# cv-core/MIT-Driverless-CV-TrainingInfra

Hardware: AMD Instinct MI355X
Metric: images/sec training (YOLOv3 416^2 + RektNet 80^2) (higher is better)
Workload: dtype bf16; 1 GPU; CVC-YOLOv3 yolo_baseline 416x416 classes=80, train step (fwd+bwd+Adam), 32 img/GPU; global_batch=32, parallelism=dp1, hipgraph=False, optimizer=FusedAdam

## Files before the change

mit-driverless-cv-traininginfra_amd/csrc/conv_igemm.hip:

```cpp
#include "conv_gemm.h"
#include "conv_shift.h"
#include "wgrad_gemm.h"
#include "wgrad_shift.h"
#include "wgrad_stream.h"

extern "C" {

static int conv2d_impl(int dtype, int mode, const void* in, int in_ldc, const void* w_packed, void* out, int out_ldc,
                       const float* bias, const void* addsrc, int add_ldc, float* stats_partial,
                       int B, int Hin, int Win, int Cin, int Hout, int Wout, int Nout,
                       int KH, int KW, int stride, int pad, int dil, const BnFuseArgs* fuse, void* stream, const EpiArgs* epi = nullptr,
                       const XAccArgs* xacc = nullptr) {
  if (!in || !w_packed || !out) return MDCV_EARG;
  if (xacc && (mode != 0 || stats_partial || fuse || epi || !xacc->acc || xacc->reps < 1 || (xacc->reps & (xacc->reps - 1)))) return MDCV_EARG;
  if (epi && (mode != 0 || stats_partial || fuse)) return MDCV_EARG;
  if ((Cin & 7) || (Nout & 7) || (in_ldc & 7) || (out_ldc & 7) || (addsrc && (add_ldc & 7))) return MDCV_EARG;
  if (stride != 1 && stride != 2) return MDCV_EARG;
  if (mode != 0 && mode != 1) return MDCV_EARG;
  ConvArgs a;
  a.in = in; a.w = w_packed; a.out = out; a.bias = bias; a.addsrc = addsrc; a.stats = stats_partial;
  a.in_ldc = in_ldc; a.out_ldc = out_ldc; a.add_ldc = add_ldc;
  a.Hin = Hin; a.Win = Win; a.Cin = Cin; a.Hout = Hout; a.Wout = Wout; a.Nout = Nout;
  a.KH = KH; a.KW = KW; a.stride = stride; a.pad = pad; a.dil = dil;
  a.M = B * Hout * Wout; a.Ktot = KH * KW * Cin; a.tiles_n = 0; a.sshift = stride == 2 ? 1 : 0; a.tiles_total = 0; a.xcd_chunk = 0;
// ... 50 lines not shown
    return dtype == MDCV_BF16 ? mdcv_cd_bf16_dgrad(a, st, B) : (dtype == MDCV_F32 ? mdcv_cd_f32_dgrad(a, st, B) : MDCV_EARG);
  }
  if (shift_ok && stats_partial) {
    const int r0 = cdiv(a.M, 128), r1 = mdcv_shift_fwd_stats_rows(B, Hout, Wout, Nout, dil);
    if (r1 > r0) {
      hipError_t e = hipMemsetAsync(stats_partial + (size_t)r0 * 2 * Nout, 0, (size_t)(r1 - r0) * 2 * Nout * sizeof(float), st);
      if (e != hipSuccess) return (int)e;
    }
  }
  if (dtype == MDCV_BF16) return mode == 0 ? mdcv_cd_bf16_fwd(a, st, B) : mdcv_cd_bf16_dgrad(a, st, B);
  if (dtype == MDCV_F32) return mode == 0 ? mdcv_cd_f32_fwd(a, st, B) : mdcv_cd_f32_dgrad(a, st, B);
  return MDCV_EARG;
}

int mdcv_conv2d(int dtype, int mode, const void* in, int in_ldc, const void* w_packed, void* out, int out_ldc,
                const float* bias, const void* addsrc, int add_ldc, float* stats_partial,
                int B, int Hin, int Win, int Cin, int Hout, int Wout, int Nout,
                int KH, int KW, int stride, int pad, int dil, void* stream) {
  MDCV_TUNE_ENTRY(dtype, MDCV_TUNE_CONV);
  return conv2d_impl(dtype, mode, in, in_ldc, w_packed, out, out_ldc, bias, addsrc, add_ldc, stats_partial, B, Hin, Win, Cin, Hout, Wout, Nout,
                     KH, KW, stride, pad, dil, nullptr, stream);
}

int mdcv_xstats_words(int reps, int C) { return reps * XACC_DIGITS * 2 * C; }
int mdcv_conv2d_xstats(int dtype, const void* in, int in_ldc, const void* w_packed, void* out, int out_ldc, const float* bias, void* xacc,
                       int reps, int B, int Hin, int Win, int Cin, int Hout, int Wout, int Nout, int KH, int KW, int stride, int pad, int dil,
                       void* stream) {
  MDCV_TUNE_ENTRY(dtype, MDCV_TUNE_CONV);
  const XAccArgs x{reinterpret_cast<long long*>(xacc), reps};
  return conv2d_impl(dtype, 0, in, in_ldc, w_packed, out, out_ldc, bias, nullptr, 0, nullptr, B, Hin, Win, Cin, Hout, Wout, Nout, KH, KW,
                     stride, pad, dil, nullptr, stream, nullptr, &x);
}

int mdcv_conv2d_affine_act(int dtype, const void* in, int in_ldc, const void* w_packed, void* out, int out_ldc, const float* scale,
                           const float* shift, const void* addsrc, int add_ldc, int act, float slope, int B, int Hin, int Win, int Cin,
                           int Hout, int Wout, int Nout, int KH, int KW, int stride, int pad, int dil, void* stream) {
  MDCV_TUNE_ENTRY(dtype, MDCV_TUNE_CONV);
  if (act < 0 || act > 2) return MDCV_EARG;
  const EpiArgs e{scale, act, slope};
  return conv2d_impl(dtype, 0, in, in_ldc, w_packed, out, out_ldc, shift, addsrc, add_ldc, nullptr, B, Hin, Win, Cin, Hout, Wout, Nout,
                     KH, KW, stride, pad, dil, nullptr, stream, &e);
}

int mdcv_conv2d_dgrad_bnsums_rows(int dtype, int B, int Hin, int Win, int Cin, int Hout, int Wout, int Nout, int KH, int KW, int stride,
                                  int pad, int dil, int in_ldc) {
  MDCV_TUNE_ENTRY(dtype, MDCV_TUNE_CONV);
  const int es = 2;
  if (dtype != MDCV_BF16) return 0;
  if (!conv_operands_small((long long)B * Hin * Win * in_ldc * es, (long long)Nout * KH * KW * Cin * es)) return 0;
  if (Hin == Hout && Win == Wout && mdcv_shift_eligible(dtype, B, Hout, Wout, Cin, Nout, KH, KW, stride, pad, dil, in_ldc))
    return mdcv_shift_stats_rows(B, Hout, Wout, dil, Nout);
  if (stride == 2 && dil == 1 && KH == 3 && KW == 3 && pad == 1 && Hout == 2 * Hin && Wout == 2 * Win && TUNE().conv_variant < 0 &&
      mdcv_shift_s2_dgrad_eligible(dtype, B, Hin, Win, Cin, Nout, in_ldc))
    return mdcv_shift_s2_rows(B, Hin, Win);
  if (stride == 2 && dil == 1) {
    int rows = 0;
    for (int cls = 0; cls < 4; ++cls) {
      const int ph = cls >> 1, pw = cls & 1;
      const int m = B * ((Hout - ph + 1) / 2) * ((Wout - pw + 1) / 2);
      if (m > 0) rows += cdiv(m, 128);
    }
    return rows;
  }
  return cdiv(B * Hout * Wout, 128);
}

int mdcv_conv2d_dgrad_bnsums(int dtype, const void* in, int in_ldc, const void* w_packed, void* out, int out_ldc, const void* addsrc,
                             int add_ldc, int B, int Hin, int Win, int Cin, int Hout, int Wout, int Nout, int KH, int KW, int stride,
                             int pad, int dil, const void* y, int ldy, const float* scale, const float* shift, const float* mean, int act,
                             float slope, float* partial, void* stream) {
  MDCV_TUNE_ENTRY(dtype, MDCV_TUNE_CONV);
  if (!y || !scale || !shift || !mean || !partial || (ldy & 7)) return MDCV_EARG;
  if (mdcv_conv2d_dgrad_bnsums_rows(dtype, B, Hin, Win, Cin, Hout, Wout, Nout, KH, KW, stride, pad, dil, in_ldc) <= 0) return MDCV_EARG;
  BnFuseArgs f;
  f.y = y; f.scale = scale; f.shift = shift; f.mean = mean; f.partial = partial; f.ldy = ldy; f.act = act; f.row_base = 0;
  f.slope = act == 2 ? 0.f : slope;
  return conv2d_impl(dtype, 1, in, in_ldc, w_packed, out, out_ldc, nullptr, addsrc, add_ldc, nullptr, B, Hin, Win, Cin, Hout, Wout, Nout,
                     KH, KW, stride, pad, dil, &f, stream);
}

int mdcv_conv2d_dgrad_s2_form_ok(int dtype, int B, int Hin, int Win, int Cin, int Hout, int Wout, int Nout, int KH, int KW, int stride,
                                 int pad, int dil, int in_ldc) {
  MDCV_TUNE_ENTRY(dtype, MDCV_TUNE_CONV);
  return dtype == MDCV_BF16 && stride == 2 && dil == 1 && KH == 3 && KW == 3 && pad == 1 && Hout == 2 * Hin && Wout == 2 * Win &&
         TUNE().conv_variant < 0 && (long long)B * Hin * Win * in_ldc * 2 < (1LL << 31) &&
         mdcv_shift_s2_dgrad_eligible(dtype, B, Hin, Win, Cin, Nout, in_ldc);
}

int mdcv_conv2d_stats_rows(int M) { return cdiv(M, 128); }
int mdcv_conv2d_stats_rows_geom(int dtype, int B, int Hout, int Wout, int Cin, int Nout, int KH, int KW, int stride, int pad, int dil,
                                int in_ldc) {
  MDCV_TUNE_ENTRY(dtype, MDCV_TUNE_CONV);
  if (mdcv_shift_eligible(dtype, B, Hout, Wout, Cin, Nout, KH, KW, stride, pad, dil, in_ldc)) return mdcv_shift_fwd_stats_rows(B, Hout, Wout, Nout, dil);
  return cdiv(B * Hout * Wout, 128);
}

int mdcv_conv2d_wgrad_splits(int dtype, int M, int Cout, int Ktot) {
  MDCV_TUNE_ENTRY(dtype, MDCV_TUNE_WGRAD);
  const int bp = dtype == MDCV_BF16 ? 128 : 64;
  const int tiles = cdiv(Cout, 128) * cdiv(Ktot, 128);
  const int slots = TUNE().wgrad_slots;
  int s = slots / tiles;
  const int max_s = cdiv(M, bp * 4);
  if (s > max_s) s = max_s;
  if (s < 1) s = 1;
  int pps = cdiv(cdiv(M, s), bp) * bp;
  return cdiv(M, pps);
// ... 106 lines not shown
```

mit-driverless-cv-traininginfra_amd/csrc/conv_shift.h:

```cpp
#pragma once
#include <hip/hip_runtime.h>
#include "bn_fuse.h"
#include "exact_acc.h"

struct ShiftArgs {
  const void* in; const void* w; void* out; const float* bias; const void* addsrc; float* stats;
  int in_ldc, out_ldc, add_ldc;
  int B, H, W, Cin, Nout;
  int Wq, Sq, Mq;
  int tiles_n, tiles_total, xcd_chunk;
  int p_base;
  int dil;
  BnFuseArgs fuse;
  EpiArgs epi;
  int t2d, tiles_x, tiles_y, TH;
  int nchunks, wrow, nca;
  XAccArgs xacc;
};

bool mdcv_shift_eligible(int dtype, int B, int H, int W, int Cin, int Nout, int KH, int KW, int stride, int pad, int dil, long long in_ldc);
int mdcv_shift_stats_rows(int B, int H, int W, int dil = 1, int Nout = 128);
int mdcv_shift_fwd_stats_rows(int B, int H, int W, int Nout, int dil = 1);
int mdcv_shift_conv(int mode, const void* in, int in_ldc, const void* w, void* out, int out_ldc, const float* bias, const void* addsrc,
                    int add_ldc, float* stats, int B, int H, int W, int Cin, int Nout, const BnFuseArgs* fuse, hipStream_t st,
                    const EpiArgs* epi = nullptr, int dil = 1, const XAccArgs* xacc = nullptr);
int mdcv_shift_s2_rows(int B, int H, int W);
bool mdcv_shift_s2_dgrad_eligible(int dtype, int B, int H, int W, int Cin, int Nout, long long in_ldc);
```

mit-driverless-cv-traininginfra_amd/csrc/conv_shift.hip:

```cpp
#include "common.h"
#include "conv_shift.h"
#include "bn_fuse.h"

#ifndef MDCV_SHIFT_PART
#define MDCV_SHIFT_PART 0
#endif
#if MDCV_SHIFT_PART == 0
#else
#endif
int mdcv_shift_launch_dgrad(const ShiftArgs& a, hipStream_t st, unsigned in_bytes, unsigned w_bytes);

namespace {

[[maybe_unused]] constexpr int BN = 128;
constexpr int WM = 4;
constexpr unsigned OOB = 0x80000000u;

__device__ __forceinline__ int swz(int row) { return (row >> 1) & 2; }
typedef __attribute__((address_space(3))) void lds_void_t;

#if defined(MDCV_SHIFT_TS) || defined(MDCV_SHIFT_WG)
#include <cstdio>
__device__ long long g_shift_wg[3 * 4096];
#endif
#ifdef MDCV_SHIFT_TS
__device__ long long g_shift_ts[4 * 512];
#define STS(k) do { if (ts_on && ts_i < 512) g_shift_ts[(k) * 512 + ts_i] = (long long)clock64(); } while (0)
#else
#define STS(k)
#endif

template <int N> __device__ __forceinline__ void wait_vm() { asm volatile("s_waitcnt vmcnt(%0)" ::"n"(N) : "memory"); }
template <int N> __device__ __forceinline__ void wait_vm_reads_done() { asm volatile("s_waitcnt vmcnt(%0) lgkmcnt(0)" ::"n"(N) : "memory"); }

}

template <int MODE, int BM, int NPA, int BRING, bool FUSE, int WN, bool EPI = false, int BN_ = 128, int LOOP = 0>
__global__ __launch_bounds__(WM * WN * 64) void mdcv_conv3x3_shift_kernel(ShiftArgs a, unsigned in_bytes, unsigned w_bytes) {
  constexpr int BN = BN_, BTILE = BN * 64, SROW = BN * 2 + 16;
  constexpr int NW = WM * WN, TN = BN / WN, FN = TN / 16;
  constexpr int TM = BM / WM, FM = TM / 16;
  static_assert(!FUSE || (WN == 2 && BM % 128 == 0), "the fused sums: 8 waves, one partial row per 128 positions");
  constexpr int STAGE = BM * SROW;
  constexpr int PIX_OFF = STAGE;
  constexpr int STAT_OFF = STAGE + BM * 4;
  extern __shared__ __attribute__((aligned(1024))) unsigned char smem[];
  const int ABYTES = a.nca * 1024;
  const int BBASE = 2 * ABYTES;
  const int SINK = BBASE + BRING * BTILE;

  const int logical = (int)(blockIdx.x & 7) * a.xcd_chunk + (int)(blockIdx.x >> 3);
  if (logical >= a.tiles_total) return;
  const int tid = threadIdx.x, lane = tid & 63;
  const int wave = __builtin_amdgcn_readfirstlane(tid >> 6);
  const int wm = wave / WN, wn = wave % WN;
  const int tile_m = logical / a.tiles_n, tile_n = logical % a.tiles_n;
  const int p0 = a.p_base + tile_m * BM;
  const int lrow = lane >> 2, kv = (lane & 3) ^ swz(lrow);

  unsigned avo[NPA];
#pragma unroll
  for (int k = 0; k < NPA; ++k) {
    const int j = (wave + k * NW) * 16 + lrow;
    int img, yy, xx;
    bool ok;
    if (a.t2d) {
      const int tpi = a.tiles_x * a.tiles_y;
      img = tile_m / tpi;
      const int rt = tile_m - img * tpi, ty = rt / a.tiles_x, tx = rt - ty * a.tiles_x;
      const int cy = j / a.Wq, cx = j - cy * a.Wq;
      if (MODE == 3) { yy = ty * a.TH + cy; xx = tx * (a.Wq - 1) + cx; }
      else { yy = ty * a.TH - 1 + cy; xx = tx * (a.Wq - 2) - 1 + cx; }
      ok = yy >= 0 && xx >= 0;
    } else {
      const int t = p0 + j - a.dil * (a.Wq + 1);
      ok = t >= 0 && t < a.Mq;
      const int tt = ok ? t : 0;
      img = tt / a.Sq;
      const int rem = tt - img * a.Sq;
      yy = rem / a.Wq; xx = rem - yy * a.Wq;
    }
    ok = ok && yy < a.H && xx < a.W && kv * 8 < a.Cin;
    avo[k] = ok ? (unsigned)((((img * a.H + yy) * a.W + xx) * a.in_ldc + kv * 8) * 2) : OOB;
  }
  unsigned bvo;
  {
    const int n = tile_n * BN + wave * 16 + lrow;
    bvo = (wave < BN / 16 && n < a.Nout) ? (unsigned)((n * a.wrow + kv * 8) * 2) : OOB;
  }
  const int r = lane & 15, q = lane >> 4;
  int offA[9];
#pragma unroll
  for (int tap = 0; tap < 9; ++tap) {
    const int kh = tap / 3, kw = tap - kh * 3;
    const int d = MODE == 3 ? (kh == 0 ? a.Wq : 0) + (kw == 0 ? 1 : 0)
                            : a.dil * (MODE == 0 ? kh * a.Wq + kw : (2 - kh) * a.Wq + (2 - kw));
    const int row = wm * TM + d + r;
    offA[tap] = row * 64 + ((q ^ swz(row)) << 4);
  }
  const int offB = (wn * TN + r) * 64 + ((q ^ swz(r)) << 4);

  const __amdgpu_buffer_rsrc_t rin = __builtin_amdgcn_make_buffer_rsrc(const_cast<void*>(a.in), 0, in_bytes, 0x00020000);
  const __amdgpu_buffer_rsrc_t rw = __builtin_amdgcn_make_buffer_rsrc(const_cast<void*>(a.w), 0, w_bytes, 0x00020000);
  const __amdgpu_buffer_rsrc_t rin0 = __builtin_amdgcn_make_buffer_rsrc(const_cast<void*>(a.in), 0, 0, 0x00020000);
  const __amdgpu_buffer_rsrc_t rw0 = __builtin_amdgcn_make_buffer_rsrc(const_cast<void*>(a.w), 0, 0, 0x00020000);
#define ISSUE_A(RS, CHUNK, BUF)                                                                                       \
  do {                                                                                                              \
    const int base__ = (BUF) * ABYTES;                                                                              \
    const int so__ = (CHUNK) * 64;                                                                                  \
    _Pragma("unroll") for (int k = 0; k < NPA; ++k) {                                                               \
      const int ch__ = wave + k * NW;              \
      __builtin_amdgcn_raw_ptr_buffer_load_lds(RS, (lds_void_t*)(smem + (ch__ < a.nca ? base__ + ch__ * 1024 : SINK)), 16, \
                                               (int)avo[k], so__, 0, 0);                                            \
    }                                                                                                               \
  } while (0)
#define ISSUE_B(RS, TAP, CHUNK, SLOT)                                                                               \
  __builtin_amdgcn_raw_ptr_buffer_load_lds(RS, (lds_void_t*)(smem + (wave < BN / 16 ? BBASE + (SLOT) * BTILE + wave * 1024 : SINK)), 16, (int)bvo, \
                                           ((TAP) * a.Cin + (CHUNK) * 32) * 2, 0, 0)

  constexpr int NCLS = MODE == 3 ? 4 : 1;
#define TAP_CLS(T) (MODE == 3 ? ((((T) / 3) != 1 ? 2 : 0) + (((T) % 3) != 1 ? 1 : 0)) * FM : 0)
  f32x4_t acc[NCLS * FM][FN];
#pragma unroll
  for (int i = 0; i < NCLS * FM; ++i)
#pragma unroll
    for (int j = 0; j < FN; ++j) acc[i][j] = f32x4_t{0.f, 0.f, 0.f, 0.f};

  constexpr int LA = BRING - 1;
  const int nch = a.nchunks;
#ifdef MDCV_SHIFT_TS
  const bool ts_on = logical == 300 && tid == 64 * 3;
  int ts_i = 0;
#endif
#if defined(MDCV_SHIFT_TS) || defined(MDCV_SHIFT_WG)
  if (tid == 0 && logical < 4096) {
    g_shift_wg[logical] = (long long)wall_clock64();
    unsigned hwid; asm volatile("s_getreg_b32 %0, hwreg(HW_REG_HW_ID)" : "=s"(hwid));
    unsigned xcc; asm volatile("s_getreg_b32 %0, hwreg(HW_REG_XCC_ID)" : "=s"(xcc));
    g_shift_wg[2 * 4096 + logical] = (long long)hwid | ((long long)xcc << 32);
  }
#endif
  ISSUE_A(rin, 0, 0);
#pragma unroll
  for (int t = 0; t < LA; ++t) ISSUE_B(rw, t % 9, t / 9, t);
  constexpr int PERIOD = BRING == 4 ? 4 : 2;
  static_assert((9 * PERIOD) % BRING == 0, "ring period");
  if constexpr (LOOP == 1) {
    const int grp = wave >> 2;
    wait_vm<LA - 1>();
    __builtin_amdgcn_s_barrier();
    if (grp == 1) __builtin_amdgcn_s_barrier();
    for (int c0 = 0; c0 < nch; c0 += PERIOD) {
#pragma unroll
      for (int cc = 0; cc < PERIOD; ++cc) {
        const int c = c0 + cc;
        if (c < nch) {
          const bool lastc = c == nch - 1;
          const int abase = (cc & 1) * ABYTES;
#pragma unroll
          for (int tap = 0; tap < 9; ++tap) {
            const int rslot = (cc * 9 + tap) % BRING, wslot = (cc * 9 + tap + LA) % BRING;
            bf16x8_t fa[FM], fb[FN];
            const unsigned char* pa = smem + abase + offA[tap];
            const unsigned char* pb = smem + BBASE + rslot * BTILE + offB;
#pragma unroll
            for (int j = 0; j < FN; ++j) fb[j] = *reinterpret_cast<const bf16x8_t*>(pb + j * 1024);
#pragma unroll
            for (int i = 0; i < FM; ++i) fa[i] = *reinterpret_cast<const bf16x8_t*>(pa + i * 1024);
            {
              const int t2 = (tap + LA) % 9, c2 = c + (tap + LA) / 9;
              if (tap + LA >= 9 && lastc) ISSUE_B(rw0, t2, c2, wslot);
              else ISSUE_B(rw, t2, c2, wslot);
            }
            if (tap == 0) {
// ... 30 lines not shown
      if (c < nch) {
        const bool lastc = c == nch - 1;
        const int abase = (cc & 1) * ABYTES;
#pragma unroll
        for (int tap = 0; tap < 9; ++tap) {
          const int rslot = (cc * 9 + tap) % BRING, wslot = (cc * 9 + tap + LA) % BRING;
          STS(0);
#pragma unroll
          for (int i = 0; i < NCLS * FM; ++i)
#pragma unroll
            for (int j = 0; j < FN; ++j) asm volatile("" : "+v"(acc[i][j]));
          if (tap >= 1 && tap <= LA) wait_vm_reads_done<LA - 1 + NPA>(); else wait_vm_reads_done<LA - 1>();
          STS(1);
          __builtin_amdgcn_s_barrier();
          STS(2);
          bf16x8_t fa[FM], fb[FN];
          const unsigned char* pa = smem + abase + offA[tap];
          const unsigned char* pb = smem + BBASE + rslot * BTILE + offB;
#pragma unroll
          for (int i = 0; i < FM; ++i) fa[i] = *reinterpret_cast<const bf16x8_t*>(pa + i * 1024);
#pragma unroll
          for (int j = 0; j < FN; ++j) fb[j] = *reinterpret_cast<const bf16x8_t*>(pb + j * 1024);
          {
            const int t2 = (tap + LA) % 9, c2 = c + (tap + LA) / 9;
            if (tap + LA >= 9 && lastc) ISSUE_B(rw0, t2, c2, wslot);
            else ISSUE_B(rw, t2, c2, wslot);
          }
          if (tap == 0) {
            if (lastc) ISSUE_A(rin0, c + 1, (cc + 1) & 1);
            else ISSUE_A(rin, c + 1, (cc + 1) & 1);
          }
#ifdef MDCV_SHIFT_PRIO
          __builtin_amdgcn_s_setprio(MDCV_SHIFT_PRIO);
#endif
#pragma unroll
          for (int i = 0; i < FM; ++i)
#pragma unroll
            for (int j = 0; j < FN; ++j) acc[TAP_CLS(tap) + i][j] = __builtin_amdgcn_mfma_f32_16x16x32_bf16(fa[i], fb[j], acc[TAP_CLS(tap) + i][j], 0, 0, 0);
#ifdef MDCV_SHIFT_PRIO
          __builtin_amdgcn_s_setprio(0);
#endif
          STS(3);
#ifdef MDCV_SHIFT_TS
          ++ts_i;
#endif
        }
      }
    }
  }
  }
  wait_vm<0>();
  __syncthreads();

  if constexpr (MODE == 3) {
    static_assert(MODE != 3 || (BM == 256 && !EPI), "stride-2 data gradient: 8 x 32 dY positions per tile");
    const int tpi = a.tiles_x * a.tiles_y;
    const int img = tile_m / tpi, rt = tile_m - img * tpi, ty = rt / a.tiles_x, tx = rt - ty * a.tiles_x;
    const int a0 = ty * a.TH, b0 = tx * (a.Wq - 1);
    const int Ho = 2 * a.H, Wo = 2 * a.W;
    bf16_t* __restrict__ out3 = reinterpret_cast<bf16_t*>(a.out);
    const bf16_t* __restrict__ add3 = reinterpret_cast<const bf16_t*>(a.addsrc);
    constexpr int VPRO3 = BN / 8;
    static_assert((512 * VPRO3) % (NW * 64) == 0 && (NW * 64) % VPRO3 == 0, "every thread keeps one channel vector");
    using Acc3 = BnFuseAcc<bf16_t, BN, NW * 64>;
    Acc3 fz3;
    const bf16_t* __restrict__ fy3 = reinterpret_cast<const bf16_t*>(a.fuse.y);
    if constexpr (FUSE) fz3.init(a.fuse, tile_n * BN + (tid % VPRO3) * 8, a.Nout);
#pragma unroll
    for (int py = 0; py < 2; ++py) {
#pragma unroll
      for (int px = 0; px < 2; ++px)
#pragma unroll
        for (int i = 0; i < FM; ++i)
#pragma unroll
          for (int j = 0; j < FN; ++j)
#pragma unroll
            for (int rr = 0; rr < 4; ++rr) {
              const int p = wm * TM + i * 16 + (lane >> 4) * 4 + rr, col = wn * TN + j * 16 + (lane & 15);
              const int srow = (p >> 5) * 64 + 2 * (p & 31) + px;
              reinterpret_cast<bf16_t*>(smem + srow * SROW)[col] = f2bf(acc[(2 * py + px) * FM + i][j][rr]);
            }
      __syncthreads();
      long long pixv[VPRO3]; uint4 aq[VPRO3], yq[VPRO3];
      const int cv = tid % VPRO3, n = tile_n * BN + cv * 8;
#pragma unroll
      for (int k = 0; k < VPRO3; ++k) {
        const int srow = (tid + k * NW * 64) / VPRO3;
        const int la = srow >> 6, ox = srow & 63;
        const int Y = 2 * (a0 + la) + py, X = 2 * b0 + ox;
        const bool ok = ox < 2 * (a.Wq - 1) && Y < Ho && X < Wo && n < a.Nout;
        pixv[k] = ok ? ((long long)img * Ho + Y) * Wo + X : -1;
        if (ok) {
          if (add3) aq[k] = *reinterpret_cast<const uint4*>(add3 + pixv[k] * a.add_ldc + n);
          if constexpr (FUSE) yq[k] = *reinterpret_cast<const uint4*>(fy3 + pixv[k] * a.fuse.ldy + n);
        }
      }
#pragma unroll
      for (int k = 0; k < VPRO3; ++k) {
        if (pixv[k] >= 0) {
          const int srow = (tid + k * NW * 64) / VPRO3;
          uint4 d = *reinterpret_cast<const uint4*>(smem + srow * SROW + cv * 16);
          float x[8];
          if (add3 || FUSE) ET<bf16_t>::unpack(d, x);
          if (add3) {
            float y[8];
            ET<bf16_t>::unpack(aq[k], y);
#pragma unroll
            for (int e = 0; e < 8; ++e) x[e] += y[e];
            d = ET<bf16_t>::pack(x);
            if constexpr (FUSE) ET<bf16_t>::unpack(d, x);
          }
          if constexpr (FUSE) {
            fz3.add(a.fuse, x, yq[k]);
          }
          *reinterpret_cast<uint4*>(out3 + pixv[k] * a.out_ldc + n) = d;
        }
      }
      __syncthreads();
    }
    if constexpr (FUSE) {
      static_assert(Acc3::kWaveFold, "bf16, at most 16 channel vectors per pixel");
      float* ws3 = reinterpret_cast<float*>(smem + 512 * SROW);
      fz3.fold_wave(ws3 + wave * 2 * BN, lane);
      lds_only_barrier();
      for (int t = tid; t < 2 * BN; t += NW * 64) Acc3::write_row(a.fuse, ws3, 2 * BN, t, tile_n * BN, a.Nout, tile_m);
    }
    return;
  }
  int* rowpix = reinterpret_cast<int*>(smem + PIX_OFF);
  if (tid < BM) {
    int img, y, x;
    bool ok;
    if (a.t2d) {
      const int tpi = a.tiles_x * a.tiles_y;
      img = tile_m / tpi;
      const int rt = tile_m - img * tpi, ty = rt / a.tiles_x, tx = rt - ty * a.tiles_x;
      const int ly = tid / a.Wq, lx = tid - ly * a.Wq;
      y = ty * a.TH + ly; x = tx * (a.Wq - 2) + lx;
      ok = lx < a.Wq - 2 && ly < a.TH;
    } else {
      const int p = p0 + tid;
      ok = p < a.Mq;
      const int pp = ok ? p : 0;
      img = pp / a.Sq;
// ... 147 lines not shown
          if (addsrc) {
            float y[8];
            ET<bf16_t>::unpack(aq[gi][u], y);
#pragma unroll
            for (int e = 0; e < 8; ++e) x[e] += y[e];
            d = ET<bf16_t>::pack(x);
            ET<bf16_t>::unpack(d, x);
          }
          *reinterpret_cast<uint4*>(out + ((size_t)pixv[gi][u] * a.out_ldc + n)) = d;
          fz.add(a.fuse, x, yq[gi][u]);
        }
      }
      if (p0 + g0 < a.Mq) {
        if constexpr (Acc::kWaveFold)
          fz.fold_wave(reinterpret_cast<float*>(smem + (g0 + wave * Acc::WROWS) * SROW), lane);
        else
          fz.flush(a.fuse, fred, tid, tile_n * BN, a.Nout, (p0 + g0) >> 7);
      }
    }
    if constexpr (Acc::kWaveFold) {
      static_assert(Acc::WROWS * SROW >= 2 * BN * 4 && SROW % 4 == 0, "a wave's dead staging rows hold its 2*BN sums");
      lds_only_barrier();
      for (int t = tid; t < NG * 2 * BN; t += NW * 64) {
        const int gi = t / (2 * BN), g0 = gi * 128;
        if (p0 + g0 < a.Mq)
          Acc::write_row(a.fuse, reinterpret_cast<const float*>(smem + g0 * SROW), Acc::WROWS * SROW / 4, t - gi * 2 * BN, tile_n * BN, a.Nout, (p0 + g0) >> 7);
      }
    }
  }
#if defined(MDCV_SHIFT_TS) || defined(MDCV_SHIFT_WG)
  if (tid == 0 && logical < 4096) g_shift_wg[4096 + logical] = (long long)wall_clock64();
#endif
}

namespace {

template <int MODE, int BM, int NPA, bool FUSE, int WN, bool EPI = false, int BRING = 3, int BN_ = 128, int LOOP = 0>
int launch_shift_f(ShiftArgs a, int p_base, int tiles_m, hipStream_t st, unsigned in_bytes, unsigned w_bytes) {
  constexpr int NW = WM * WN;
  constexpr int BN = BN_, BTILE = BN * 64, SROW = BN * 2 + 16;
  if constexpr (LOOP == 0 && WN == 2 && !EPI && MODE == 0 && !FUSE) {
    if (TUNE().shift_loop == 1 || BM > 256 || (TUNE().shift_loop == 2 && tiles_m * a.tiles_n <= 256))
      return launch_shift_f<MODE, BM, NPA, FUSE, WN, EPI, BRING, BN_, 1>(a, p_base, tiles_m, st, in_bytes, w_bytes);
  }
  if constexpr (BRING == 3 && WN == 2 && !EPI) {
    if ((TUNE().shift_ring == 4 && tiles_m * a.tiles_n <= 256) || TUNE().shift_ring == 5)
      return launch_shift_f<MODE, BM, NPA, FUSE, WN, EPI, 4, BN_, LOOP>(a, p_base, tiles_m, st, in_bytes, w_bytes);
  }
  a.p_base = p_base;
  a.tiles_total = tiles_m * a.tiles_n;
  a.xcd_chunk = (a.tiles_total + 7) / 8;
  a.nca = (BM + 2 * a.dil * (a.Wq + 1) + 15) / 16;
  const int pipe = 2 * a.nca * 1024 + BRING * BTILE + 1024;
  const int epi = MODE == 3 ? 512 * SROW + NW * 2 * BN * 4
                            : BM * SROW + BM * 4 + WM * 2 * BN * 4;
  const int lds = pipe > epi ? pipe : epi;
  static DynLds dyn_lds;
  auto kern = mdcv_conv3x3_shift_kernel<MODE, BM, NPA, BRING, FUSE, WN, EPI, BN_, LOOP>;
  if (hipError_t e = mdcv_dyn_lds(dyn_lds, reinterpret_cast<const void*>(kern), lds); e != hipSuccess) return (int)e;
  MDCV_LAUNCH(kern, dim3((unsigned)(a.xcd_chunk * 8)), dim3(NW * 64), lds, st, a, in_bytes, w_bytes);
  MDCV_CHECK_LAUNCH();
  return MDCV_OK;
}

template <int MODE, int BM, int NPA, int WN, int BN_>
int launch_shift(const ShiftArgs& a, int p_base, int tiles_m, hipStream_t st, unsigned in_bytes, unsigned w_bytes) {
  if constexpr (MODE == 3) {
    if (a.fuse.y) return launch_shift_f<MODE, BM, NPA, true, WN, false, 3, BN_>(a, p_base, tiles_m, st, in_bytes, w_bytes);
  }
  if constexpr (MODE == 1 && WN == 2 && BM % 128 == 0) {
    if (a.fuse.y) return launch_shift_f<MODE, BM, NPA, true, WN, false, 3, BN_>(a, p_base, tiles_m, st, in_bytes, w_bytes);
  }
  if constexpr (MODE == 0 && WN == 2) {
    if (a.epi.oscale || a.epi.act) return launch_shift_f<MODE, BM, NPA, false, WN, true, 3, BN_>(a, p_base, tiles_m, st, in_bytes, w_bytes);
  }
  if (a.epi.oscale || a.epi.act) return MDCV_EARG;
  return launch_shift_f<MODE, BM, NPA, false, WN, false, 3, BN_>(a, p_base, tiles_m, st, in_bytes, w_bytes);
}

template <int MODE, int BM, int BN_>
int launch_shift_bm(const ShiftArgs& a, int p_base, int tiles_m, hipStream_t st, unsigned in_bytes, unsigned w_bytes) {
  const int nca = (BM + 2 * a.dil * (a.Wq + 1) + 15) / 16;
  const int npa = (nca + 7) / 8;
  if (npa <= 2) return launch_shift<MODE, BM, 2, 2, BN_>(a, p_base, tiles_m, st, in_bytes, w_bytes);
  if (npa == 3) return launch_shift<MODE, BM, 3, 2, BN_>(a, p_base, tiles_m, st, in_bytes, w_bytes);
  if (npa == 4) return launch_shift<MODE, BM, 4, 2, BN_>(a, p_base, tiles_m, st, in_bytes, w_bytes);
  return launch_shift<MODE, BM, 5, 2, BN_>(a, p_base, tiles_m, st, in_bytes, w_bytes);
}

int shift_plan_bm(int Mq, int tiles_n, bool fused, int halo = 0, int bn = 128, bool fwd = false) {
  if (halo > 0 && !fused && 2 * ((256 + halo + 15) / 16) * 1024 + 3 * bn * 64 + 1024 > 80 * 1024) {
    for (int bm = 256; bm >= 128; bm -= 64) {
      const int nca = (bm + halo + 15) / 16;
      if (2 * nca * 1024 + 3 * bn * 64 + 1024 <= 80 * 1024) return bm;
    }
    return 256;
  }
  if (bn == 128 && !fused && fwd && halo <= 110) {
    const int t384 = ((Mq + 383) / 384) * tiles_n;
    if (TUNE().shift_big == 384 || (TUNE().shift_loop == 2 && t384 > 192 && t384 <= 256)) return 384;
  }
  if (TUNE().shift_plan == 1) return 256;
  if (TUNE().shift_plan == 2) return 128;
  const int t256 = ((Mq + 255) / 256) * tiles_n;
  if (t256 <= 128) return 128;
  if (fused || TUNE().shift_plan == 6) return 256;
  const int t192 = ((Mq + 191) / 192) * tiles_n;
  const int c256 = ((t256 + 255) / 256) * 256, c192 = ((t192 + 255) / 256) * 192;
  return c192 < c256 ? 192 : 256;
}

template <int MODE, int BN_>
int launch_shift_mode(const ShiftArgs& a, hipStream_t st, unsigned in_bytes, unsigned w_bytes) {
  if constexpr (MODE == 3) {
    return launch_shift_bm<MODE, 256, BN_>(a, 0, a.Mq / 256, st, in_bytes, w_bytes);
  } else {
  if (a.t2d) return launch_shift_bm<MODE, 256, BN_>(a, 0, a.Mq / 256, st, in_bytes, w_bytes);
  const int bm = shift_plan_bm(a.Mq, a.tiles_n, a.fuse.y != nullptr, 2 * a.dil * (a.Wq + 1), BN_, MODE == 0);
  if constexpr (BN_ == 128 && MODE == 0) {
    if (bm == 384) return launch_shift_bm<MODE, 384, BN_>(a, 0, (a.Mq + 383) / 384, st, in_bytes, w_bytes);
  }
  if (bm == 192) return launch_shift_bm<MODE, 192, BN_>(a, 0, (a.Mq + 191) / 192, st, in_bytes, w_bytes);
  const int big_m = (a.Mq + 255) / 256;
  const int nbig_m = bm == 128 ? 0 : big_m;
  if (nbig_m > 0) {
    const int rc = launch_shift_bm<MODE, 256, BN_>(a, 0, nbig_m, st, in_bytes, w_bytes);
    if (rc) return rc;
  }
  const int p_base = nbig_m * 256;
  if (p_base < a.Mq) return launch_shift_bm<MODE, 128, BN_>(a, p_base, (a.Mq - p_base + 127) / 128, st, in_bytes, w_bytes);
  return MDCV_OK;
  }
}

}

#if MDCV_SHIFT_PART == 1
int mdcv_shift_launch_dgrad(const ShiftArgs& a, hipStream_t st, unsigned in_bytes, unsigned w_bytes) {
  if (a.t2d == 2) {
    if (a.Nout == 32) return launch_shift_mode<3, 32>(a, st, in_bytes, w_bytes);
    if (a.Nout == 64) return launch_shift_mode<3, 64>(a, st, in_bytes, w_bytes);
    return MDCV_EARG;
  }
  if (a.Nout == 32) return launch_shift_mode<1, 32>(a, st, in_bytes, w_bytes);
  if (a.Nout == 64) return launch_shift_mode<1, 64>(a, st, in_bytes, w_bytes);
  if (TUNE().shift_n64_wide && !a.t2d && a.Nout % 64 == 0 && ((a.Mq + 255) / 256) * a.tiles_n <= 128) {
    ShiftArgs b = a;
    b.tiles_n = a.Nout / 64;
    return launch_shift_mode<1, 64>(b, st, in_bytes, w_bytes);
  }
  return launch_shift_mode<1, 128>(a, st, in_bytes, w_bytes);
}
#else
static bool shift_fits_1d(int W, int Nout) {
  return W <= TUNE().shift_wmax || (TUNE().shift_wmax_narrow && Nout <= 64 && W <= TUNE().shift_wmax_narrow) || (TUNE().shift_wmax_n32 && Nout <= 32 && W <= TUNE().shift_wmax_n32);
}
static bool shift_is_2d(int W, int Nout, int dil) { return dil == 1 && TUNE().shift_2d && !shift_fits_1d(W, Nout); }
constexpr int T2D_WQ = 32, T2D_TH = 8;
static long long shift_2d_positions(int B, int H, int W) { return (long long)B * ((H + T2D_TH - 1) / T2D_TH) * ((W + T2D_WQ - 3) / (T2D_WQ - 2)) * 256; }

bool mdcv_shift_eligible(int dtype, int B, int H, int W, int Cin, int Nout, int KH, int KW, int stride, int pad, int dil, long long in_ldc) {
  if (dtype != MDCV_BF16 || KH != 3 || KW != 3 || stride != 1 || pad != dil || (dil != 1 && !(dil == 2 && TUNE().shift_dil2))) return false;
  if (dil == 2 && TUNE().shift_dil2 == 1 && !(Nout <= 64 && Cin >= 64)) return false;
  if ((Cin & 31) || ((Nout & 127) && !(Nout == 64 && TUNE().shift_n64) && !(Nout == 32 && TUNE().shift_n64 == 2))) return false;
  if (H < 8 || W < 8) return false;
  if (!shift_fits_1d(W, Nout) && !(TUNE().shift_2d && dil == 1)) return false;
  if ((long long)B * (H + dil) * (W + dil) + 1024 >= (1LL << 30) || shift_2d_positions(B, H, W) >= (1LL << 30)) return false;
  if ((long long)B * H * W * in_ldc * 2 >= (1LL << 31) || (long long)Nout * 9 * Cin * 2 >= (1LL << 31)) return false;
  return true;
}

bool mdcv_shift_s2_dgrad_eligible(int dtype, int B, int H, int W, int Cin, int Nout, long long in_ldc) {
  if (!TUNE().shift_s2 || dtype != MDCV_BF16 || (Cin & 31) || Cin < 32 || !(Nout == 32 || Nout == 64) || H < 1 || W < 1) return false;
  if ((long long)B * ((H + 7) / 8) * ((W + 30) / 31) * 256 >= (1LL << 30)) return false;
  if ((long long)B * H * W * in_ldc * 2 >= (1LL << 31) || (long long)Nout * 9 * Cin * 2 >= (1LL << 31)) return false;
  return true;
}

int mdcv_shift_s2_rows(int B, int H, int W) { return B * ((H + T2D_TH - 1) / T2D_TH) * ((W + T2D_WQ - 2) / (T2D_WQ - 1)); }

int mdcv_shift_stats_rows(int B, int H, int W, int dil, int Nout) {
  if (shift_is_2d(W, Nout, dil)) return (int)(shift_2d_positions(B, H, W) / 128);
  return (int)(((long long)B * (H + dil) * (W + dil) + 127) / 128);
}
int mdcv_shift_fwd_stats_rows(int B, int H, int W, int Nout, int dil) {
  if (shift_is_2d(W, Nout, dil)) return (int)(shift_2d_positions(B, H, W) / 128);
  const int Mq = B * (H + dil) * (W + dil);
  const int bn = Nout <= 64 ? Nout : BN;
  const int bm = shift_plan_bm(Mq, Nout <= 64 ? 1 : Nout / BN, false, 2 * dil * (W + dil + 1), bn, true);
  return (bm == 192 || bm == 384) ? (Mq + bm - 1) / bm : (Mq + 127) / 128;
}

int mdcv_shift_conv(int mode, const void* in, int in_ldc, const void* w, void* out, int out_ldc, const float* bias, const void* addsrc,
                    int add_ldc, float* stats, int B, int H, int W, int Cin, int Nout, const BnFuseArgs* fuse, hipStream_t st,
                    const EpiArgs* epi, int dil, const XAccArgs* xacc) {
  ShiftArgs a;
  a.xacc = XAccArgs{nullptr, 1};
  if (xacc) { if (mode != 0 || stats || epi || !xacc->acc || xacc->reps < 1 || (xacc->reps & (xacc->reps - 1))) return MDCV_EARG; a.xacc = *xacc; }
  if (fuse) a.fuse = *fuse; else a.fuse = BnFuseArgs{};
  if (epi) a.epi = *epi; else a.epi = EpiArgs{nullptr, 0, 0.f};
  a.in = in; a.w = w; a.out = out; a.bias = bias; a.addsrc = addsrc; a.stats = stats;
  a.in_ldc = in_ldc; a.out_ldc = out_ldc; a.add_ldc = add_ldc;
  a.B = B; a.H = H; a.W = W; a.Cin = Cin; a.Nout = Nout;
  a.dil = dil; a.Wq = W + dil; a.Sq = (H + dil) * (W + dil); a.Mq = B * a.Sq;
  a.t2d = 0; a.tiles_x = a.tiles_y = a.TH = 0;
  if (mode == 3) {
    a.t2d = 2; a.Wq = T2D_WQ; a.TH = T2D_TH;
    a.tiles_x = (W + T2D_WQ - 2) / (T2D_WQ - 1); a.tiles_y = (H + T2D_TH - 1) / T2D_TH;
    a.Mq = B * a.tiles_x * a.tiles_y * 256; a.Sq = a.tiles_x * a.tiles_y * 256;
  } else if (shift_is_2d(W, Nout, dil)) {
    a.t2d = 1; a.Wq = T2D_WQ; a.TH = T2D_TH;
    a.tiles_x = (W + T2D_WQ - 3) / (T2D_WQ - 2); a.tiles_y = (H + T2D_TH - 1) / T2D_TH;
    a.Mq = (int)shift_2d_positions(B, H, W); a.Sq = a.tiles_x * a.tiles_y * 256;
  }
  a.tiles_n = Nout <= 64 ? 1 : Nout / BN;
  a.tiles_total = 0; a.xcd_chunk = 0; a.nca = 0; a.p_base = 0;
  a.nchunks = (Cin + 31) / 32;
  a.wrow = 9 * Cin;
  const unsigned in_bytes = (unsigned)((long long)B * H * W * in_ldc * 2);
  const unsigned w_bytes = (unsigned)((long long)Nout * 9 * Cin * 2);
  if (mode == 3 && (epi || stats || bias)) return MDCV_EARG;
  if (mode != 0) return mdcv_shift_launch_dgrad(a, st, in_bytes, w_bytes);
  if (Nout == 32) return launch_shift_mode<0, 32>(a, st, in_bytes, w_bytes);
  if (Nout == 64) return launch_shift_mode<0, 64>(a, st, in_bytes, w_bytes);
  return launch_shift_mode<0, 128>(a, st, in_bytes, w_bytes);
}

#ifdef MDCV_SHIFT_TS
extern "C" int mdcv_debug_shift_ts(long long* host4x512) {
  return (int)hipMemcpyFromSymbol(host4x512, HIP_SYMBOL(g_shift_ts), sizeof(long long) * 4 * 512);
}
#endif
#if defined(MDCV_SHIFT_TS) || defined(MDCV_SHIFT_WG)
extern "C" int mdcv_debug_shift_occ(int lds) {
  int nb = -1;
  auto kern = mdcv_conv3x3_shift_kernel<0, 256, 3, 3, false, 2>;
  hipFuncSetAttribute(reinterpret_cast<const void*>(kern), hipFuncAttributeMaxDynamicSharedMemorySize, lds);
  hipError_t e = hipOccupancyMaxActiveBlocksPerMultiprocessor(&nb, reinterpret_cast<const void*>(kern), 512, (size_t)lds);
  hipFuncAttributes fa; hipFuncGetAttributes(&fa, reinterpret_cast<const void*>(kern));
  printf("occupancy(lds=%d) = %d blocks/CU (err %d); numRegs %d sharedSizeBytes %zu maxThreadsPerBlock %d\n", lds, nb, (int)e, fa.numRegs,
         (size_t)fa.sharedSizeBytes, fa.maxThreadsPerBlock);
  return nb;
}
extern "C" int mdcv_debug_shift_wg(long long* host3x4096) {
  return (int)hipMemcpyFromSymbol(host3x4096, HIP_SYMBOL(g_shift_wg), sizeof(long long) * 3 * 4096);
}
#endif

#endif
```

mit-driverless-cv-traininginfra_amd/csrc/tune.h:

```cpp
#pragma once

struct MdcvTune {
  int conv_no_ut = 0;
  int conv_tall_narrow = 256;
  int conv_deep_narrow = 1;
  int conv_deep_small = 8;
  int conv_fuse_narrow = 1;
  int conv_variant = -1;
  int conv_tall_s2 = 1;
  int conv_deep_s2 = 1;
  int conv_s2_allcls = 1;
  int conv_s2_split = 512;
  int conv_s2_split_on = 1;
  int wgrad_slots = 512;
  int wgrad_bna_stages = 2;
  int wgrad_variant = 0;
  int shift_ring = 4;
  int shift_wmax_narrow = 104;
  int shift_wmax_n32 = 0;
  int shift_dil2 = 1;
  int shift_n64 = 2;
  int shift_wmax = 80;
  int shift_loop = 2;
  int shift_2d = 1;
  int shift_big = 0;
  int shift_n64_wide = 1;
  int shift_plan = 0;
  int shift_s2 = 1;
  int pw_bmp = 0;
  int pw_wres = 1;
  int stream_blocks = 0;
  int stream_tiled = 1;
  int stream_light_maxpos = 600000;
  int stream_table = 1;
  int stream_direct = 1;
  int stream_s2 = 1;
  int stream_s2_blocks = 256;
  int stream_s2_depth = 2;
  int stream_s2_lds = 160 * 1024;
  int stream_light_depth = 1;
  int stream_light_blocks = 256;
  int stream_tiled_blocks = 128;
};

extern thread_local const MdcvTune* mdcv_t_tune;
inline const MdcvTune& TUNE() { return *mdcv_t_tune; }

enum { MDCV_TUNE_CONV = 0, MDCV_TUNE_WGRAD = 1, MDCV_TUNE_PW = 2 };

inline void mdcv_tune_shift(MdcvTune& t, int ring) {
  if (ring == 63 || ring == 64) { t.shift_n64_wide = ring - 63; return; }
  if (ring == 29 || ring == 60) { t.shift_s2 = ring == 60; return; }
  if (ring == 27 || ring == 28) { t.shift_2d = ring - 27; return; }
  if (ring >= 200 && ring < 300) { t.shift_big = ring == 201 ? 384 : 0; return; }
  if (ring >= 30 && ring <= 59) { t.shift_loop = ring - 30; return; }
  if (ring == 25 || ring == 26) { t.shift_wmax_n32 = ring == 25 ? 208 : 0; return; }
  if (ring == 23 || ring == 24) { t.shift_wmax_narrow = ring == 23 ? 104 : 0; return; }
  if (ring >= 20 && ring <= 22) { t.shift_dil2 = ring == 20 ? 2 : (ring == 21 ? 0 : 1); return; }
  if (ring >= 17 && ring <= 19) { t.shift_n64 = ring == 17 ? 1 : (ring == 18 ? 0 : 2); return; }
  if (ring >= 14 && ring <= 16) { t.shift_wmax = ring == 14 ? 80 : (ring == 15 ? 62 : 104); return; }
  if (ring >= 7) t.shift_plan = ring - 7;
  else if (ring >= 3 && ring <= 5) t.shift_ring = ring;
}
inline void mdcv_tune_apply_conv(MdcvTune& t, int v) {
  if (v == 0) return;
  if (v <= -3 && v >= -299) { mdcv_tune_shift(t, -v); return; }
  if (v == 93 || v == 92) { t.conv_fuse_narrow = v == 93; return; }
  if (v >= 60 && v < 92) { t.conv_deep_small = v - 60; return; }
  if (v >= 30 && v < 60) { t.conv_deep_narrow = v - 30; return; }
  if (v == 20 || v == 21) { t.conv_deep_s2 = v - 20; return; }
  if (v == 16 || v == 17) { t.conv_s2_allcls = v - 16; return; }
  if (v == 14 || v == 15) { t.conv_s2_split_on = v - 14; return; }
  if (v >= 4000 && v < 6000) { t.conv_s2_split = v - 4000; return; }
  if (v == 18 || v == 19) { t.conv_tall_s2 = v - 18; return; }
  if (v >= 2000 && v < 3000) { t.conv_tall_narrow = v - 2000; return; }
  if (v >= 100) { t.conv_no_ut = 1; v -= 100; }
  if (v >= 1 && v <= 12) t.conv_variant = v - 1;
}
inline void mdcv_tune_apply_wgrad(MdcvTune& t, int v) {
  if (v == 0) return;
  if (v >= 20000 && v < 30000) { t.wgrad_slots = v - 20000; return; }
  if (v >= 35000 && v < 36000) { t.stream_s2_blocks = v - 35000; return; }
  if (v >= 30000 && v < 40000) {
    const int b = v - 30000;
    if (b >= 4001 && b <= 4002) { t.stream_light_depth = b - 4000; return; }
    if (b >= 4012 && b <= 4014) { t.wgrad_bna_stages = b - 4010; return; }
    if (b == 4020 || b == 4021) { t.stream_table = b - 4020; return; }
    if (b == 4050 || b == 4051) { t.stream_direct = b - 4050; return; }
    if (b == 4060 || b == 4061) { t.stream_s2 = b - 4060; return; }
    if (b >= 4071 && b <= 4073) { t.stream_s2_depth = b - 4070; return; }
    if (b >= 4100 && b <= 4260) { t.stream_s2_lds = (b - 4100) * 1024; return; }
    if (b == 2) t.stream_light_maxpos = 600000;
    else if (b == 3) t.stream_light_maxpos = 1 << 30;
    else if (b == 5) t.stream_light_maxpos = 0;
    else if (b >= 3000 && b < 4000) t.stream_light_blocks = b - 3000;
    else t.stream_tiled_blocks = b > 0 ? b : 128;
    return;
  }
  if (v >= 1000) { const int d = (v - 1000) / 100; t.stream_tiled = !(d & 8); t.stream_blocks = ((v - 1000) % 100) * 64; return; }
  t.wgrad_variant = v;
}
inline void mdcv_tune_apply_pw(MdcvTune& t, int v) {
  if (v == 1000 || v == 1001) { t.pw_wres = v - 1000; return; }
  if (v == 64 || v == 32 || v == 16) t.pw_bmp = v;
}
// ... 21 lines not shown
```

Measured before the change: 2491 images/sec.

## Add wide-channel stride-2 shift dgrad mode using flat tiling and pixel table

Adds a new MODE 4 path to the shift-conv kernel for stride-2 3x3 data-gradient convolutions with Nout above 64 (multiples of 64, width up to 62). It uses flat position tiling instead of 2D tiles, plus an LDS pixel table that maps each dY position to its output base address for the four-class scatter epilogue. Previously these wider layers fell back to the generic per-class igemm path. The new path is enabled by default behind a tune knob, with a minimum position count. It raises LDS usage and adds a template instantiation.

Result: no change. 2502 images/sec (median of 6 runs) (+0.4%).

```diff
diff --git a/mit-driverless-cv-traininginfra_amd/csrc/conv_igemm.hip b/mit-driverless-cv-traininginfra_amd/csrc/conv_igemm.hip
--- a/mit-driverless-cv-traininginfra_amd/csrc/conv_igemm.hip
+++ b/mit-driverless-cv-traininginfra_amd/csrc/conv_igemm.hip
@@ -126,7 +126,7 @@
     return mdcv_shift_stats_rows(B, Hout, Wout, dil, Nout);
   if (stride == 2 && dil == 1 && KH == 3 && KW == 3 && pad == 1 && Hout == 2 * Hin && Wout == 2 * Win && TUNE().conv_variant < 0 &&
       mdcv_shift_s2_dgrad_eligible(dtype, B, Hin, Win, Cin, Nout, in_ldc))
-    return mdcv_shift_s2_rows(B, Hin, Win);
+    return mdcv_shift_s2_rows(B, Hin, Win, Nout);
   if (stride == 2 && dil == 1) {
     int rows = 0;
     for (int cls = 0; cls < 4; ++cls) {
diff --git a/mit-driverless-cv-traininginfra_amd/csrc/conv_shift.h b/mit-driverless-cv-traininginfra_amd/csrc/conv_shift.h
--- a/mit-driverless-cv-traininginfra_amd/csrc/conv_shift.h
+++ b/mit-driverless-cv-traininginfra_amd/csrc/conv_shift.h
@@ -24,5 +24,5 @@
 int mdcv_shift_conv(int mode, const void* in, int in_ldc, const void* w, void* out, int out_ldc, const float* bias, const void* addsrc,
                     int add_ldc, float* stats, int B, int H, int W, int Cin, int Nout, const BnFuseArgs* fuse, hipStream_t st,
                     const EpiArgs* epi = nullptr, int dil = 1, const XAccArgs* xacc = nullptr);
-int mdcv_shift_s2_rows(int B, int H, int W);
+int mdcv_shift_s2_rows(int B, int H, int W, int Nout);
 bool mdcv_shift_s2_dgrad_eligible(int dtype, int B, int H, int W, int Cin, int Nout, long long in_ldc);
diff --git a/mit-driverless-cv-traininginfra_amd/csrc/conv_shift.hip b/mit-driverless-cv-traininginfra_amd/csrc/conv_shift.hip
--- a/mit-driverless-cv-traininginfra_amd/csrc/conv_shift.hip
+++ b/mit-driverless-cv-traininginfra_amd/csrc/conv_shift.hip
@@ -64,7 +64,7 @@
     const int j = (wave + k * NW) * 16 + lrow;
     int img, yy, xx;
     bool ok;
-    if (a.t2d) {
+    if (MODE != 4 && a.t2d) {
       const int tpi = a.tiles_x * a.tiles_y;
       img = tile_m / tpi;
       const int rt = tile_m - img * tpi, ty = rt / a.tiles_x, tx = rt - ty * a.tiles_x;
@@ -73,7 +73,7 @@
       else { yy = ty * a.TH - 1 + cy; xx = tx * (a.Wq - 2) - 1 + cx; }
       ok = yy >= 0 && xx >= 0;
     } else {
-      const int t = p0 + j - a.dil * (a.Wq + 1);
+      const int t = MODE == 4 ? p0 + j : p0 + j - a.dil * (a.Wq + 1);
       ok = t >= 0 && t < a.Mq;
       const int tt = ok ? t : 0;
       img = tt / a.Sq;
@@ -93,7 +93,7 @@
 #pragma unroll
   for (int tap = 0; tap < 9; ++tap) {
     const int kh = tap / 3, kw = tap - kh * 3;
-    const int d = MODE == 3 ? (kh == 0 ? a.Wq : 0) + (kw == 0 ? 1 : 0)
+    const int d = MODE >= 3 ? (kh == 0 ? a.Wq : 0) + (kw == 0 ? 1 : 0)
                             : a.dil * (MODE == 0 ? kh * a.Wq + kw : (2 - kh) * a.Wq + (2 - kw));
     const int row = wm * TM + d + r;
     offA[tap] = row * 64 + ((q ^ swz(row)) << 4);
@@ -118,8 +118,8 @@
   __builtin_amdgcn_raw_ptr_buffer_load_lds(RS, (lds_void_t*)(smem + (wave < BN / 16 ? BBASE + (SLOT) * BTILE + wave * 1024 : SINK)), 16, (int)bvo, \
                                            ((TAP) * a.Cin + (CHUNK) * 32) * 2, 0, 0)
 
-  constexpr int NCLS = MODE == 3 ? 4 : 1;
-#define TAP_CLS(T) (MODE == 3 ? ((((T) / 3) != 1 ? 2 : 0) + (((T) % 3) != 1 ? 1 : 0)) * FM : 0)
+  constexpr int NCLS = MODE >= 3 ? 4 : 1;
+#define TAP_CLS(T) (MODE >= 3 ? ((((T) / 3) != 1 ? 2 : 0) + (((T) % 3) != 1 ? 1 : 0)) * FM : 0)
   f32x4_t acc[NCLS * FM][FN];
 #pragma unroll
   for (int i = 0; i < NCLS * FM; ++i)
@@ -256,12 +256,27 @@
   wait_vm<0>();
   __syncthreads();
 
-  if constexpr (MODE == 3) {
-    static_assert(MODE != 3 || (BM == 256 && !EPI), "stride-2 data gradient: 8 x 32 dY positions per tile");
-    const int tpi = a.tiles_x * a.tiles_y;
-    const int img = tile_m / tpi, rt = tile_m - img * tpi, ty = rt / a.tiles_x, tx = rt - ty * a.tiles_x;
-    const int a0 = ty * a.TH, b0 = tx * (a.Wq - 1);
+  if constexpr (MODE >= 3) {
+    static_assert(MODE < 3 || (BM == 256 && !EPI), "stride-2 data gradient: 256 dY positions per tile");
     const int Ho = 2 * a.H, Wo = 2 * a.W;
+    int img = 0, a0 = 0, b0 = 0;
+    [[maybe_unused]] int* pixtab = reinterpret_cast<int*>(smem + 512 * SROW + NW * 2 * BN * 4);
+    if constexpr (MODE == 3) {
+      const int tpi = a.tiles_x * a.tiles_y;
+      img = tile_m / tpi;
+      const int rt = tile_m - img * tpi, ty = rt / a.tiles_x, tx = rt - ty * a.tiles_x;
+      a0 = ty * a.TH; b0 = tx * (a.Wq - 1);
+    } else {
+      if (tid < BM) {
+        const int t = p0 + tid;
+        int base = -1;
+        if (t < a.Mq) {
+          const int im = t / a.Sq, rem = t - im * a.Sq, ya = rem / a.Wq, xb = rem - ya * a.Wq;
+          if (ya < a.H && xb < a.W) base = (im * Ho + 2 * ya) * Wo + 2 * xb;
+        }
+        pixtab[tid] = base;
+      }
+    }
     bf16_t* __restrict__ out3 = reinterpret_cast<bf16_t*>(a.out);
     const bf16_t* __restrict__ add3 = reinterpret_cast<const bf16_t*>(a.addsrc);
     constexpr int VPRO3 = BN / 8;
@@ -290,10 +305,17 @@
 #pragma unroll
       for (int k = 0; k < VPRO3; ++k) {
         const int srow = (tid + k * NW * 64) / VPRO3;
-        const int la = srow >> 6, ox = srow & 63;
-        const int Y = 2 * (a0 + la) + py, X = 2 * b0 + ox;
-        const bool ok = ox < 2 * (a.Wq - 1) && Y < Ho && X < Wo && n < a.Nout;
-        pixv[k] = ok ? ((long long)img * Ho + Y) * Wo + X : -1;
+        bool ok;
+        if constexpr (MODE == 3) {
+          const int la = srow >> 6, ox = srow & 63;
+          const int Y = 2 * (a0 + la) + py, X = 2 * b0 + ox;
+          ok = ox < 2 * (a.Wq - 1) && Y < Ho && X < Wo && n < a.Nout;
+          pixv[k] = ok ? ((long long)img * Ho + Y) * Wo + X : -1;
+        } else {
+          const int base = pixtab[srow >> 1];
+          ok = base >= 0 && n < a.Nout;
+          pixv[k] = ok ? (long long)(base + py * Wo + (srow & 1)) : -1;
+        }
         if (ok) {
           if (add3) aq[k] = *reinterpret_cast<const uint4*>(add3 + pixv[k] * a.add_ldc + n);
           if constexpr (FUSE) yq[k] = *reinterpret_cast<const uint4*>(fy3 + pixv[k] * a.fuse.ldy + n);
@@ -547,7 +569,7 @@
   a.xcd_chunk = (a.tiles_total + 7) / 8;
   a.nca = (BM + 2 * a.dil * (a.Wq + 1) + 15) / 16;
   const int pipe = 2 * a.nca * 1024 + BRING * BTILE + 1024;
-  const int epi = MODE == 3 ? 512 * SROW + NW * 2 * BN * 4
+  const int epi = MODE >= 3 ? 512 * SROW + NW * 2 * BN * 4 + (MODE == 4 ? 256 * 4 : 0)
                             : BM * SROW + BM * 4 + WM * 2 * BN * 4;
   const int lds = pipe > epi ? pipe : epi;
   static DynLds dyn_lds;
@@ -560,7 +582,7 @@
 
 template <int MODE, int BM, int NPA, int WN, int BN_>
 int launch_shift(const ShiftArgs& a, int p_base, int tiles_m, hipStream_t st, unsigned in_bytes, unsigned w_bytes) {
-  if constexpr (MODE == 3) {
+  if constexpr (MODE >= 3) {
     if (a.fuse.y) return launch_shift_f<MODE, BM, NPA, true, WN, false, 3, BN_>(a, p_base, tiles_m, st, in_bytes, w_bytes);
   }
   if constexpr (MODE == 1 && WN == 2 && BM % 128 == 0) {
@@ -577,10 +599,14 @@
 int launch_shift_bm(const ShiftArgs& a, int p_base, int tiles_m, hipStream_t st, unsigned in_bytes, unsigned w_bytes) {
   const int nca = (BM + 2 * a.dil * (a.Wq + 1) + 15) / 16;
   const int npa = (nca + 7) / 8;
+  if constexpr (MODE == 4) {
+    return npa <= 3 ? launch_shift<MODE, BM, 3, 2, BN_>(a, p_base, tiles_m, st, in_bytes, w_bytes) : MDCV_EARG;
+  } else {
   if (npa <= 2) return launch_shift<MODE, BM, 2, 2, BN_>(a, p_base, tiles_m, st, in_bytes, w_bytes);
   if (npa == 3) return launch_shift<MODE, BM, 3, 2, BN_>(a, p_base, tiles_m, st, in_bytes, w_bytes);
   if (npa == 4) return launch_shift<MODE, BM, 4, 2, BN_>(a, p_base, tiles_m, st, in_bytes, w_bytes);
   return launch_shift<MODE, BM, 5, 2, BN_>(a, p_base, tiles_m, st, in_bytes, w_bytes);
+  }
 }
 
 int shift_plan_bm(int Mq, int tiles_n, bool fused, int halo = 0, int bn = 128, bool fwd = false) {
@@ -609,6 +635,8 @@
 int launch_shift_mode(const ShiftArgs& a, hipStream_t st, unsigned in_bytes, unsigned w_bytes) {
   if constexpr (MODE == 3) {
     return launch_shift_bm<MODE, 256, BN_>(a, 0, a.Mq / 256, st, in_bytes, w_bytes);
+  } else if constexpr (MODE == 4) {
+    return launch_shift_bm<MODE, 256, BN_>(a, 0, (a.Mq + 255) / 256, st, in_bytes, w_bytes);
   } else {
   if (a.t2d) return launch_shift_bm<MODE, 256, BN_>(a, 0, a.Mq / 256, st, in_bytes, w_bytes);
   const int bm = shift_plan_bm(a.Mq, a.tiles_n, a.fuse.y != nullptr, 2 * a.dil * (a.Wq + 1), BN_, MODE == 0);
@@ -632,6 +660,7 @@
 
 #if MDCV_SHIFT_PART == 1
 int mdcv_shift_launch_dgrad(const ShiftArgs& a, hipStream_t st, unsigned in_bytes, unsigned w_bytes) {
+  if (a.t2d == 3) return launch_shift_mode<4, 64>(a, st, in_bytes, w_bytes);
   if (a.t2d == 2) {
     if (a.Nout == 32) return launch_shift_mode<3, 32>(a, st, in_bytes, w_bytes);
     if (a.Nout == 64) return launch_shift_mode<3, 64>(a, st, in_bytes, w_bytes);
@@ -665,14 +694,27 @@
   return true;
 }
 
+constexpr int S2_WIDE_WMAX = 62;
+constexpr long long S2_WIDE_MIN_POS = 4096;
+static bool shift_s2_is_wide(int Nout) { return Nout > 64; }
 bool mdcv_shift_s2_dgrad_eligible(int dtype, int B, int H, int W, int Cin, int Nout, long long in_ldc) {
-  if (!TUNE().shift_s2 || dtype != MDCV_BF16 || (Cin & 31) || Cin < 32 || !(Nout == 32 || Nout == 64) || H < 1 || W < 1) return false;
-  if ((long long)B * ((H + 7) / 8) * ((W + 30) / 31) * 256 >= (1LL << 30)) return false;
+  if (!TUNE().shift_s2 || dtype != MDCV_BF16 || (Cin & 31) || Cin < 32 || H < 1 || W < 1) return false;
+  if (shift_s2_is_wide(Nout)) {
+    if (!TUNE().shift_s2_wide || (Nout & 63) || W > S2_WIDE_WMAX) return false;
+    if (TUNE().shift_s2_wide == 1 && (long long)B * H * W < S2_WIDE_MIN_POS) return false;
+    if ((long long)B * (H + 1) * (W + 1) + 1024 >= (1LL << 30)) return false;
+  } else {
+    if (!(Nout == 32 || Nout == 64)) return false;
+    if ((long long)B * ((H + 7) / 8) * ((W + 30) / 31) * 256 >= (1LL << 30)) return false;
+  }
   if ((long long)B * H * W * in_ldc * 2 >= (1LL << 31) || (long long)Nout * 9 * Cin * 2 >= (1LL << 31)) return false;
   return true;
 }
 
-int mdcv_shift_s2_rows(int B, int H, int W) { return B * ((H + T2D_TH - 1) / T2D_TH) * ((W + T2D_WQ - 2) / (T2D_WQ - 1)); }
+int mdcv_shift_s2_rows(int B, int H, int W, int Nout) {
+  if (shift_s2_is_wide(Nout)) return (int)(((long long)B * (H + 1) * (W + 1) + 255) / 256);
+  return B * ((H + T2D_TH - 1) / T2D_TH) * ((W + T2D_WQ - 2) / (T2D_WQ - 1));
+}
 
 int mdcv_shift_stats_rows(int B, int H, int W, int dil, int Nout) {
   if (shift_is_2d(W, Nout, dil)) return (int)(shift_2d_positions(B, H, W) / 128);
@@ -699,7 +741,9 @@
   a.B = B; a.H = H; a.W = W; a.Cin = Cin; a.Nout = Nout;
   a.dil = dil; a.Wq = W + dil; a.Sq = (H + dil) * (W + dil); a.Mq = B * a.Sq;
   a.t2d = 0; a.tiles_x = a.tiles_y = a.TH = 0;
-  if (mode == 3) {
+  if (mode == 3 && shift_s2_is_wide(Nout)) {
+    a.t2d = 3;
+  } else if (mode == 3) {
     a.t2d = 2; a.Wq = T2D_WQ; a.TH = T2D_TH;
     a.tiles_x = (W + T2D_WQ - 2) / (T2D_WQ - 1); a.tiles_y = (H + T2D_TH - 1) / T2D_TH;
     a.Mq = B * a.tiles_x * a.tiles_y * 256; a.Sq = a.tiles_x * a.tiles_y * 256;
@@ -708,7 +752,7 @@
     a.tiles_x = (W + T2D_WQ - 3) / (T2D_WQ - 2); a.tiles_y = (H + T2D_TH - 1) / T2D_TH;
     a.Mq = (int)shift_2d_positions(B, H, W); a.Sq = a.tiles_x * a.tiles_y * 256;
   }
-  a.tiles_n = Nout <= 64 ? 1 : Nout / BN;
+  a.tiles_n = Nout <= 64 ? 1 : (a.t2d == 3 ? Nout / 64 : Nout / BN);
   a.tiles_total = 0; a.xcd_chunk = 0; a.nca = 0; a.p_base = 0;
   a.nchunks = (Cin + 31) / 32;
   a.wrow = 9 * Cin;
diff --git a/mit-driverless-cv-traininginfra_amd/csrc/tune.h b/mit-driverless-cv-traininginfra_amd/csrc/tune.h
--- a/mit-driverless-cv-traininginfra_amd/csrc/tune.h
+++ b/mit-driverless-cv-traininginfra_amd/csrc/tune.h
@@ -27,6 +27,7 @@
   int shift_n64_wide = 1;
   int shift_plan = 0;
   int shift_s2 = 1;
+  int shift_s2_wide = 1;
   int pw_bmp = 0;
   int pw_wres = 1;
   int stream_blocks = 0;
@@ -51,6 +52,7 @@
 inline void mdcv_tune_shift(MdcvTune& t, int ring) {
   if (ring == 63 || ring == 64) { t.shift_n64_wide = ring - 63; return; }
   if (ring == 29 || ring == 60) { t.shift_s2 = ring == 60; return; }
+  if (ring == 61 || ring == 62) { t.shift_s2_wide = ring == 62 ? 2 : 0; return; }
   if (ring == 27 || ring == 28) { t.shift_2d = ring - 27; return; }
   if (ring >= 200 && ring < 300) { t.shift_big = ring == 201 ? 384 : 0; return; }
   if (ring >= 30 && ring <= 59) { t.shift_loop = ring - 30; return; }
```
